# HKUST-Aerial-Robotics/MIND

Measured on AMD Instinct MI355X. Metric: sim steps/sec (whole node) + scenario-tree nodes expanded/sec, AV2 demo scenes, higher is better.
Workload: dtype f32-class (bf16 hi+mid+lo split operands = 24 significand bits, six products, fp32 accumulate) pair kernel + ActorNet, f32 elsewhere in the predictor, f64 iLQR

## Files before the change

include/mind_hip.h:

```cpp
#ifndef MIND_HIP_H
#define MIND_HIP_H

#include <stddef.h>
#include <stdint.h>

#ifdef __cplusplus
extern "C" {
#endif

#define MIND_OK 0
#define MIND_EINVAL (-1)
#define MIND_ENOMEM (-2)
#define MIND_EHIP (-3)
#define MIND_ESTATE (-4)
#define MIND_ENOTFOUND (-5)

typedef struct mind_ctx mind_ctx;

int mind_ctx_create(int device, void *stream, mind_ctx **out);
int mind_ctx_destroy(mind_ctx *ctx);
const char *mind_last_error_string(mind_ctx *ctx);
int mind_ctx_synchronize(mind_ctx *ctx);

typedef struct {
// ... 84 lines not shown
int mind_debug_aime_book(int pred_len, int max_depth, int max_rounds, int n_agents, int world, int rank, int force, int n_rounds, const int *dec_len,
                         const float *dec, int n_tokens, int bytes_per_pair, int plan_chunk_mb, int per_scene, long long *out, int cap, char *msg,
                         int msg_cap);

int mind_debug_wait_word(const unsigned *word, unsigned want, double timeout_s, double (*clock)(void *user), void *user, int spins_per_look);

int mind_debug_actor_lw_plan(int n_actors, int np, int chunk, long long *out_launches, int cap, long long *out_info);

int mind_debug_token_lw_plan(int n_tokens, int mode, int chunk, long long *out_launches, int cap, long long *out_info);

int mind_debug_pack_conv_frag(const float *w, int co, int ci, int ksz, uint32_t *out, size_t cap);

int mind_debug_pack(const char *what, const float *w, int a, int b, int c, float *out, size_t cap);
int mind_debug_weight_image(const mind_tensor_desc *tensors, int n_tensors, float *blob, size_t blob_cap, char *names, size_t names_cap,
                            long long *entries, int entries_cap, long long *out_info, char *msg, int msg_cap);
int mind_debug_weight_bind(const mind_tensor_desc *tensors, int n_tensors, const char *drop, char *msg, int msg_cap);

int mind_debug_trig(mind_ctx *ctx, const double *x, int n, double *out);

int mind_debug_dec_scene(mind_ctx *ctx, const float *rows, int n_scenes, int form, float *Cout, float *cls, int reps, float *ms);

int mind_debug_set_layers(mind_ctx *ctx, int n);
int64_t mind_debug_read(mind_ctx *ctx, const char *name, float *host, int64_t max_floats);

typedef struct {
  int n_nodes;
  const int32_t *parent;
  const float *prob;
  int n_agents;
  const float *agent_mean;
  const float *agent_cov;
  const double *field;
  const double *node_w;
} mind_cost_tree;

typedef struct {
  double dt, wheelbase;
  double w_des_state[6];
  double w_state_con[6];
  double state_lower[6], state_upper[6];
  double w_ctrl[2];
  double w_tgt, w_ego, w_ego_cov_offset, w_exo, w_exo_cov_offset, w_exo_cost_offset;
  double grid_res; int grid_w, grid_h;
  int max_iter;
} mind_ilqr_cfg;

// ... 362 lines not shown
```

mind_amd/_lib.py:

```python
import ctypes as C
import os

_HERE = os.path.dirname(os.path.abspath(__file__))
LIB_PATH = os.environ.get("MIND_HIP_LIB", os.path.join(_HERE, "libmind_hip.so"))

WAIT_CLOCK = C.CFUNCTYPE(C.c_double, C.c_void_p)
MIND_OK = 0
MIND_EINVAL, MIND_ENOMEM, MIND_EHIP, MIND_ESTATE, MIND_ENOTFOUND = -1, -2, -3, -4, -5


class TensorDesc(C.Structure):
    _fields_ = [("name", C.c_char_p), ("data", C.POINTER(C.c_float)), ("numel", C.c_int64)]


class SceneBatch(C.Structure):
    _fields_ = [("n_scenes", C.c_int), ("actor_off", C.POINTER(C.c_int32)), ("lane_off", C.POINTER(C.c_int32)),
                ("actors", C.c_void_p), ("lanes", C.c_void_p), ("lane_feat", C.c_void_p),
                ("actor_ctrs", C.c_void_p), ("actor_vecs", C.c_void_p), ("lane_ctrs", C.c_void_p),
                ("lane_vecs", C.c_void_p), ("rpe", C.POINTER(C.c_void_p)), ("tgt_nodes", C.c_void_p),
                ("tgt_rpe", C.c_void_p)]


class PredOut(C.Structure):
    _fields_ = [("cls", C.c_void_p), ("reg", C.c_void_p), ("vel", C.c_void_p), ("lane_feat", C.c_void_p),
# ... 177 lines not shown
                ("n_agents", C.c_int), ("n_trees", C.c_int), ("best", C.c_int), ("n_expanded", C.c_int), ("n_rounds", C.c_int), ("n_traj_nodes", C.c_int),
                ("costs", C.POINTER(C.c_double)), ("aime_s", C.c_double), ("ilqr_s", C.c_double), ("total_s", C.c_double),
                ("tot", LoopTotals)]


PLANNER_EGO_KEY = -(1 << 63)


class PlannerDesc(C.Structure):
    _fields_ = [("time_ahead", C.c_double), ("min_vel", C.c_float), ("dist_thres", C.c_float), ("max_depth", C.c_int), ("max_rounds", C.c_int),
                ("pred_len", C.c_int), ("prob_floor", C.c_float), ("cfg_warm", C.c_void_p), ("cfg_full", C.c_void_p), ("speculative", C.c_int),
                ("ego_type_slot", C.c_int)]


class PlannerOut(C.Structure):
    _fields_ = [("n_plans", C.c_longlong),
                ("n_agents", C.c_int), ("n_trees", C.c_int), ("best", C.c_int), ("n_expanded", C.c_int), ("n_rounds", C.c_int), ("n_traj_nodes", C.c_int),
                ("costs", C.POINTER(C.c_double)), ("ctrl", C.c_double * 2), ("aime_s", C.c_double), ("ilqr_s", C.c_double), ("total_s", C.c_double),
                ("tot", LoopTotals)]


EXPORTS = ["mind_ctx_create", "mind_ctx_destroy", "mind_last_error_string", "mind_ctx_synchronize",
           "mind_weights_load", "mind_predict_batch", "mind_last_fusion_stats", "mind_last_actor_stats", "mind_debug_actor_lw_plan", "mind_last_token_stats", "mind_last_token_stage_ms", "mind_debug_token_lw_plan", "mind_set_profiling", "mind_debug_launch_times", "mind_debug_launch_clock",
           "mind_ilqr_solve_trees", "mind_ilqr_contingency", "mind_ilqr_solve_fields", "mind_cost_eval", "mind_ilqr_score_trees", "mind_ilqr_gains", "mind_ilqr_policy_rollouts", "mind_lane_dist_field", "mind_aime_world", "mind_aime_rebase", "mind_debug_aime_decide", "mind_debug_set_layers",
           "mind_debug_read", "mind_set_pair_precision", "mind_get_pair_precision", "mind_debug_pack_bfrag", "mind_debug_pack_conv_frag", "mind_debug_pack", "mind_debug_weight_image", "mind_debug_weight_bind", "mind_debug_pair_schedule", "mind_debug_predict_choice", "mind_debug_ilqr_plan", "mind_debug_aime_book", "mind_set_tuning", "mind_get_tuning", "mind_debug_tuning", "mind_debug_live_handles", "mind_last_ilqr_stats", "mind_aime_plan", "mind_last_ilqr_profile", "mind_eval_traj_trees", "mind_last_ilqr_trace", "mind_ilqr_contingency_begin", "mind_ilqr_finish", "mind_fill_tracks", "mind_ilqr_contingency_begin_plan", "mind_debug_trig", "mind_aime_plan_begin", "mind_aime_plan_poll", "mind_aime_plan_finish", "mind_ctx_busy", "mind_ilqr_finish_plan", "mind_debug_dec_scene",
           "mind_set_exchange", "mind_last_exchange_stats", "mind_debug_wait_word",
           "mind_predict_batch_aux", "mind_set_decoder_basis", "mind_get_decoder_basis", "mind_curve_eval", "mind_debug_curve_basis",
           "mind_audit_plan", "mind_audit_episode", "mind_debug_box_clearance",
           "mind_forecast_score", "mind_debug_forecast_score",
           "mind_audit_road_plan", "mind_audit_road_episode", "mind_debug_road_margin",
           "mind_audit_ttc", "mind_debug_box_ttc",
           "mind_loop_create", "mind_loop_destroy", "mind_loop_reset", "mind_loop_advance", "mind_loop_state", "mind_loop_last_plan", "mind_loop_export",
           "mind_planner_create", "mind_planner_destroy", "mind_planner_reset", "mind_planner_observe", "mind_planner_set_lanes", "mind_planner_set_target_lane",
           "mind_planner_set_solve_lane", "mind_planner_set_eval_lane", "mind_planner_plan", "mind_planner_last_plan", "mind_planner_export"]

EXCHANGE_FN = C.CFUNCTYPE(C.c_int, C.c_void_p, C.c_int, C.c_void_p, C.c_void_p, C.c_int64)
XCHG_ALLGATHER, XCHG_ALLREDUCE, XCHG_ALLTOALLV = 0, 1, 2

_lib = None


def load():
    global _lib
    if _lib is not None:
        return _lib
    if not os.path.exists(LIB_PATH):
        raise ImportError(f"{LIB_PATH} is missing: the HIP extension must be built (hipcc --offload-arch=gfx950); "
# ... 71 lines not shown
    lib.mind_debug_live_handles.argtypes = []
    lib.mind_last_ilqr_stats.argtypes = [C.c_void_p, C.POINTER(C.c_float), C.POINTER(C.c_int), C.POINTER(C.c_int)]
    lib.mind_last_ilqr_profile.argtypes = [C.c_void_p, C.POINTER(C.c_double)]
    lib.mind_last_ilqr_trace.argtypes = [C.c_void_p, C.c_int, C.c_int, C.POINTER(C.c_double), C.c_int, C.POINTER(C.c_int)]
    lib.mind_eval_traj_trees.argtypes = [C.POINTER(C.c_double), C.POINTER(C.c_double), C.POINTER(C.c_int32), C.c_int, C.c_void_p, C.c_int, C.c_int,
                                         C.c_double, C.POINTER(C.c_double)]
    lib.mind_get_pair_precision.argtypes = [C.c_void_p]
    lib.mind_debug_pack_bfrag.argtypes = [C.POINTER(C.c_float), C.c_int, C.POINTER(C.c_uint32)]
    lib.mind_debug_pair_schedule.argtypes = [C.POINTER(C.c_int), C.POINTER(C.c_int), C.c_int, C.c_int, C.c_int, C.POINTER(C.c_int), C.c_int, C.POINTER(C.c_int)]
    lib.mind_debug_predict_choice.argtypes = [C.POINTER(C.c_char_p), C.POINTER(C.c_int), C.c_int, C.c_int, C.c_int, C.c_int, C.POINTER(C.c_int), C.POINTER(C.c_int),
                                              C.c_int, C.POINTER(C.c_longlong), C.c_int]
    lib.mind_debug_ilqr_plan.argtypes = [C.POINTER(C.c_char_p), C.POINTER(C.c_int), C.c_int, C.c_int, C.c_int, C.c_int, C.POINTER(C.c_int), C.POINTER(C.c_int32),
                                         C.POINTER(C.c_longlong), C.c_int, C.POINTER(C.c_int)]
    lib.mind_debug_wait_word.argtypes = [C.POINTER(C.c_uint), C.c_uint, C.c_double, WAIT_CLOCK, C.c_void_p, C.c_int]
    lib.mind_debug_aime_book.argtypes = [C.c_int] * 8 + [C.POINTER(C.c_int), C.POINTER(C.c_float)] + [C.c_int] * 4 + [C.POINTER(C.c_longlong), C.c_int, C.c_char_p, C.c_int]
    lib.mind_debug_trig.argtypes = [C.c_void_p, C.POINTER(C.c_double), C.c_int, C.POINTER(C.c_double)]
    lib.mind_debug_pack_conv_frag.argtypes = [C.POINTER(C.c_float), C.c_int, C.c_int, C.c_int, C.POINTER(C.c_uint32), C.c_size_t]
    lib.mind_debug_pack.argtypes = [C.c_char_p, C.POINTER(C.c_float), C.c_int, C.c_int, C.c_int, C.POINTER(C.c_float), C.c_size_t]
    lib.mind_debug_weight_image.argtypes = [C.POINTER(TensorDesc), C.c_int, C.POINTER(C.c_float), C.c_size_t, C.c_char_p, C.c_size_t,
                                            C.POINTER(C.c_longlong), C.c_int, C.POINTER(C.c_longlong), C.c_char_p, C.c_int]
    lib.mind_debug_weight_bind.argtypes = [C.POINTER(TensorDesc), C.c_int, C.c_char_p, C.c_char_p, C.c_int]
    lib.mind_debug_dec_scene.argtypes = [C.c_void_p, C.POINTER(C.c_float), C.c_int, C.c_int, C.POINTER(C.c_float), C.POINTER(C.c_float), C.c_int, C.POINTER(C.c_float)]
    lib.mind_debug_set_layers.argtypes = [C.c_void_p, C.c_int]
    lib.mind_debug_read.argtypes = [C.c_void_p, C.c_char_p, C.POINTER(C.c_float), C.c_int64]
    lib.mind_set_exchange.argtypes = [C.c_void_p, C.c_int, C.c_int, EXCHANGE_FN, C.c_void_p, C.c_int]
    lib.mind_last_exchange_stats.argtypes = [C.c_void_p, C.POINTER(C.c_longlong), C.POINTER(C.c_longlong)]
    lib.mind_loop_create.argtypes = [C.c_void_p, C.POINTER(LoopDesc), C.POINTER(C.c_void_p)]
    lib.mind_loop_destroy.argtypes = [C.c_void_p]
    lib.mind_loop_reset.argtypes = [C.c_void_p]
    lib.mind_loop_advance.argtypes = [C.c_void_p, C.c_int, C.c_double, C.c_longlong, C.POINTER(LoopOut)]
    lib.mind_loop_state.argtypes = [C.c_void_p, C.POINTER(LoopOut)]
    lib.mind_loop_last_plan.argtypes = [C.c_void_p, C.POINTER(AimePlanOut)] + [C.POINTER(C.c_void_p)] * 6 + [C.c_void_p]
    lib.mind_loop_export.argtypes = [C.c_void_p, C.c_int, C.POINTER(C.c_int), C.c_void_p, C.c_void_p, C.c_void_p]
    lib.mind_planner_create.argtypes = [C.c_void_p, C.POINTER(PlannerDesc), C.POINTER(C.c_void_p)]
    lib.mind_planner_destroy.argtypes = [C.c_void_p]
    lib.mind_planner_reset.argtypes = [C.c_void_p]
    lib.mind_planner_observe.argtypes = [C.c_void_p, C.c_int, C.c_void_p, C.c_int, C.c_void_p, C.c_void_p, C.c_void_p]
    lib.mind_planner_set_lanes.argtypes = [C.c_void_p, C.c_int, C.c_void_p, C.c_void_p]
    lib.mind_planner_set_target_lane.argtypes = [C.c_void_p, C.c_int, C.c_void_p, C.c_void_p]
    lib.mind_planner_set_solve_lane.argtypes = [C.c_void_p, C.c_int, C.c_void_p, C.c_double]
    lib.mind_planner_set_eval_lane.argtypes = [C.c_void_p, C.c_int, C.c_void_p, C.c_int]
    lib.mind_planner_plan.argtypes = [C.c_void_p, C.c_void_p, C.c_void_p, C.POINTER(PlannerOut)]
    lib.mind_planner_last_plan.argtypes = [C.c_void_p, C.POINTER(AimePlanOut)] + [C.POINTER(C.c_void_p)] * 6 + [C.c_void_p]
    lib.mind_planner_export.argtypes = [C.c_void_p, C.c_int, C.POINTER(C.c_int), C.c_void_p, C.c_void_p, C.c_void_p]
    lib.mind_audit_plan.argtypes = [C.c_void_p, C.POINTER(AuditBox), C.c_double, C.POINTER(CostTree), C.c_int, C.c_int, C.POINTER(C.c_double),
                                    C.POINTER(AuditPlanOut)]
# ... 28 lines not shown
                      "xcd_lanes5", "dec_actor", "dec_np", "fp32_dec", "split_dec", "want_mw", "mw_blocks", "cls_on_side", "tgt_wait_first",
                      "dec_head_ra", "dec_chain_g")
PAIR_PREC = ("f32", "bf16x3", "bf16", "bf16x6")


def predict_choice(knobs, prec, scenes, n_cu=256, have_side=True):
    lib = load()
    names = (C.c_char_p * max(1, len(knobs)))(*[k.encode() for k in knobs])
    vals = (C.c_int * max(1, len(knobs)))(*[int(v) for v in knobs.values()])
    sa = (C.c_int * len(scenes))(*[a for a, _ in scenes])
    sl = (C.c_int * len(scenes))(*[l for _, l in scenes])
    cap = 32 + 6 * len(scenes)
    out = (C.c_longlong * cap)()
    n = lib.mind_debug_predict_choice(names, vals, len(knobs), PAIR_PREC.index(prec) if isinstance(prec, str) else prec, n_cu, int(have_side),
                                      sa, sl, len(scenes), out, cap)
    if n == MIND_EINVAL:
        return None
    assert 0 < n <= cap and out[0] == 32 and n == 32 + 6 * out[1], n
    d = dict(zip(PRED_CHOICE_FIELDS, out[:32]))
    d["runs"] = [tuple(out[32 + 6 * i:38 + 6 * i]) for i in range(out[1])]
    return d


def dec_scene(lib, ctx, rows, form, reps=1, timed=False):
    import numpy as np
    rows = np.ascontiguousarray(rows, np.float32)
    B = rows.shape[0]
    assert rows.shape == (B, 128)
    fp = C.POINTER(C.c_float)
    cout, cls, ms = np.empty((B, 6, 128), np.float32), np.empty((B, 6), np.float32), np.zeros(reps, np.float32)
    check(lib, ctx, lib.mind_debug_dec_scene(ctx, rows.ctypes.data_as(fp), B, int(form), cout.ctypes.data_as(fp), cls.ctypes.data_as(fp), reps,
                                             ms.ctypes.data_as(fp) if timed else None), "mind_debug_dec_scene")
    return (cout, cls, ms) if timed else (cout, cls)


def knobs():
    lib = load()
    name, env, val = C.c_char_p(), C.c_char_p(), C.c_int()
    rows = []
    while not rows or len(rows) < n:
        n = lib.mind_debug_tuning(len(rows), None, None, 0, C.byref(name), C.byref(env), C.byref(val))
        assert n > 0, n
        rows.append((name.value.decode(), env.value.decode() if env.value else None, val.value))
    return rows


# ... 279 lines not shown
```

mind_amd/csrc/fusion_kernels.hip:

```cpp
#include <hip/hip_runtime.h>
#include <stdint.h>

#include "pair_common.h"

#define D_ 128
#define LDS_WAE 0
#define LDS_WAP 16384
#define LDS_STAGE 32768
#define LDS_PTAB (LDS_STAGE + PAIR_WAVES * STAGE_FLOATS)
#define LDS_SVEC (LDS_PTAB + PAIR_WAVES * 128)
#define LDS_VT (LDS_SVEC + PAIR_WAVES * 136)
#define LDS_RT (LDS_VT + VT_SIZE)
#define LDS_TOTAL (LDS_RT + 1024)

#define LDS_FENCE() asm volatile("s_waitcnt lgkmcnt(0)" ::: "memory")

__device__ __forceinline__ void gemm128(frag8 &acc, const float *wa, const frag8 &bsrc, int lane) {
  int lo = lane * 4;
  OPAQUE(lo);
  const float *wl = wa + lo;
  f32x4 c0 = *(const f32x4 *)(wl + (0 * 8 + 0) * 256);
  f32x4 c1 = *(const f32x4 *)(wl + (1 * 8 + 0) * 256);
#pragma unroll
  for (int st = 0; st < 32; ++st) {
// ... 626 lines not shown
  TT(7);
#ifdef MIND_TOKEN_TRACE
  if (blockIdx.x == 0 && tid == 0)
    printf("[k_token mode %d ntok %d] cycles: load %lld cw %lld combine %lld Wv %lld Wo+LN2 %lld FFN+LN3 %lld S,T,q %lld QK %lld\n", mode, n_tok,
           tt_[0], tt_[1], tt_[2], tt_[3], tt_[4], tt_[5], tt_[6], tt_[7]);
#endif
}

template <int TPW>
__global__ __launch_bounds__(TT_THREADS) __attribute__((amdgpu_waves_per_eu(4, 4))) void k_token(const TokMeta *__restrict__ meta, int n_tok, int mode,
                                                      const float *__restrict__ actor_feat,
                                                      const float *__restrict__ lane_feat, float *__restrict__ x,
                                                      const float *__restrict__ part, float *__restrict__ ST,
                                                      float *__restrict__ QK, TokWeights W) {
  k_token_body<TPW, false>(meta, n_tok, mode, actor_feat, lane_feat, x, part, ST, QK, W);
}
__global__ __launch_bounds__(TT_THREADS) __attribute__((amdgpu_waves_per_eu(2, 2))) void k_token_m(const TokMeta *__restrict__ meta, int n_tok, int mode,
                                                      const float *__restrict__ actor_feat,
                                                      const float *__restrict__ lane_feat, float *__restrict__ x,
                                                      const float *__restrict__ part, float *__restrict__ ST,
                                                      float *__restrict__ QK, TokWeights W) {
  k_token_body<TOK_TPW_SMALL, true>(meta, n_tok, mode, actor_feat, lane_feat, x, part, ST, QK, W);
}
```

mind_amd/csrc/mind_hip.hip:

```cpp
#include <hip/hip_runtime.h>

#include <cmath>
#include <cstdarg>
#include <cstdio>
#include <cstdlib>
#include <algorithm>
#include <cstring>
#include <map>
#include <memory>
#include <string>
#include <thread>
#include <atomic>
#include <functional>
#include <vector>

#include "../../include/mind_hip.h"
#include "encdec_kernels.hip"
#include "fusion_kernels.hip"
#include "pair_bf16_kernels.hip"
#include "pair_tile_kernels.hip"
#include "pair_tile6_kernels.hip"
#include "token_mfma_kernels.hip"
#include "actor_mfma_kernels.hip"
#include "actor_lw_kernels.hip"
// ... 149 lines not shown
  Event ev_rows;
  std::vector<const double *> il_trace_dev;
  std::vector<int> il_trace_its;
  int il_trace_cap = 0, il_trace_phases = 0;
  double il_prof[9] = {0, 0, 0, 0, 0, 0, 0, 0, 0};
  long long n_ilqr_fallbacks = 0;
  int n_pair_launch = 0;
  float pair_ms = 0.f;
  double pairs_done = 0.0;
  std::vector<Event> ev;
  bool ev_defer = false;
  std::vector<Event> ev_pool;
  size_t ev_pool_used = 0;
  std::vector<size_t> ev_pending;
  int wall_khz = 0;
  LcRing lc;
  DevBuf lc_dev;
  Pinned lc_host;
  double lc_carry_ms[LC_KINDS] = {0, 0, 0};
  int lc_carry_n[LC_KINDS] = {0, 0, 0};
  std::vector<float> lc_last[LC_KINDS], ev_last[LC_KINDS];
  int n_cu = 256;
  int debug_layers = 6;
  int last_ntok = 0;
  size_t il_dbg[6] = {0, 0, 0, 0, 0, 0};
  long long last_edge_pairs = 0;
  int last_slots = 0, last_A = 0, last_B = 0;
};

static int fail(mind_ctx *c, int code, const char *fmt, ...) {
  char buf[512];
  va_list ap;
  va_start(ap, fmt);
  vsnprintf(buf, sizeof(buf), fmt, ap);
  va_end(ap);
  if (c) c->err = buf;
  return code;
}

#define HIPCHK(c, call)                                                                        \
  do {                                                                                         \
    hipError_t e_ = (call);                                                                    \
    if (e_ != hipSuccess)                                                                      \
      return fail(c, MIND_EHIP, "%s failed: %s (%s:%d)", #call, hipGetErrorString(e_), __FILE__, __LINE__); \
  } while (0)

// ... 977 lines not shown
```

mind_amd/csrc/pred_choice.h:

```cpp
#pragma once
#include <vector>

#include "tuning.h"
#include "dec_chain.h"

static inline int pred_mfma_parts(const PredTuning &t, int pair_prec) {
  return (pair_prec == 3 || (pair_prec == 1 && t.actor_np == 6)) ? 6 : (pair_prec == 1 ? 3 : 1);
}

static inline bool pred_edge_tiled(const PredTuning &t, int pair_prec) { return pair_prec == 3 || (pair_prec != 0 && t.pair_tile); }

static inline int pred_edge_pair_bytes(const PredTuning &t, int pair_prec) { return pred_edge_tiled(t, pair_prec) && pair_prec == 2 ? 256 : 512; }

enum PredActorForm { PRED_ACTOR_VALU = 0, PRED_ACTOR_F32 = 1, PRED_ACTOR_MFMA = 2, PRED_ACTOR_LW = 3 };
enum PredPairFamily { PRED_PAIR_F32 = 0, PRED_PAIR_BF = 1, PRED_PAIR_T = 2, PRED_PAIR_T6 = 3 };
enum PredDecActor { PRED_DEC_ONE = 0, PRED_DEC_SPLIT = 1, PRED_DEC_MFMA = 2 };

struct PredTokRun {
  int t0, n, kind;
  bool layerwise;
  bool small, merged;
};

struct PredChoice {
  int np = 1;
  int actor_form = PRED_ACTOR_VALU, actor_arg = 0, actor_grid = 0, actor_chunk = 0, actor_chunks = 1, actor_launches = 1;
  int qsplit = 0, qk_stride = 1024;
  bool tiled = false, edge_bf16 = false;
  std::vector<PredTokRun> tok_runs;
  int tok_chunk = 0;
  bool tok_lw = false;
  int last_tok_chunks = 0;
  int pair_family = PRED_PAIR_F32, pair_np = 0;
  bool l5_jobs5 = false;
  int xcd_lanes = 1, xcd_lanes5 = 1;
  int dec_actor = PRED_DEC_ONE;
  int dec_head_ra = RA;
  bool fp32_dec = true, split_dec = false, want_mw = false, cls_side = false;
  int mw_blocks = 0;
  int dec_chain_g = 0;
  bool tgt_wait_first = false;
};

static PredChoice pred_choose(const PredTuning &t, int pair_prec, int n_cu, bool have_side, int n_scenes, const int *scene_actors, const int *scene_lanes) {
  PredChoice ch;
  int A = 0;
  for (int b = 0; b < n_scenes; ++b) A += scene_actors[b];
  ch.np = pred_mfma_parts(t, pair_prec);

  ch.actor_grid = A;
  if (t.actor_f32 && A >= (pair_prec == 0 ? t.actor_f32_pair_min : t.actor_f32_min)) {
    ch.actor_form = PRED_ACTOR_F32; ch.actor_arg = 2; ch.actor_grid = (A + 1) / 2;
  } else if (pair_prec == 0 && t.actor_f32 && t.enc_mfma) {
    ch.actor_form = PRED_ACTOR_F32; ch.actor_arg = 1;
  } else if (pair_prec == 0 || !t.enc_mfma) {
    ch.actor_form = PRED_ACTOR_VALU;
  } else if (A >= t.actor_lw_min) {
    ch.actor_form = PRED_ACTOR_LW; ch.actor_arg = ch.np;
    ch.actor_chunk = t.actor_lw_chunk > 0 ? t.actor_lw_chunk : LW_CHUNK;
    ch.actor_chunks = (A + ch.actor_chunk - 1) / ch.actor_chunk;
    ch.actor_grid = ch.actor_chunks;
    ch.actor_launches = ch.actor_chunks * (1 + 2 * LW_NSTAGE);
  } else {
    ch.actor_form = PRED_ACTOR_MFMA; ch.actor_arg = ch.np;
  }

  ch.qsplit = pair_prec == 3 ? 48 : pair_prec != 0 ? 16 : 0;
  ch.qk_stride = pair_prec == 3 ? P6_QK_STRIDE : 1024;
  ch.tiled = pred_edge_tiled(t, pair_prec);
  ch.edge_bf16 = pred_edge_pair_bytes(t, pair_prec) == 256;

  ch.tok_chunk = t.tok_lw_chunk > 0 ? t.tok_lw_chunk : TL_CHUNK;
  long long njobs = 0, njobs5 = 0;
  int t0 = 0;
  for (int b = 0; b < n_scenes; ++b) {
    const int N = scene_actors[b] + scene_lanes[b] + 1;
    const int kind = t.tok_mfma ? 1 : (pair_prec != 0 && pair_prec != 3 && t.tok_bf_min_n > 0 && N >= t.tok_bf_min_n) ? 2 : N >= t.tok_lw_min_n ? 1 : 0;
    if (!ch.tok_runs.empty() && ch.tok_runs.back().kind == kind) ch.tok_runs.back().n += N;
    else ch.tok_runs.push_back({t0, N, kind, false, false, false});
    t0 += N;
    njobs += (long long)N * pair_column_splits(N);
    njobs5 += (long long)(scene_actors[b] + 1) * pair_column_splits(N);
  }
  for (PredTokRun &r : ch.tok_runs) {
    r.layerwise = r.kind == 1 && r.n >= t.tok_lw_min;
    r.small = r.kind == 0 && r.n <= t.tok_small_max;
    r.merged = r.small && t.tok_merge;
    if (r.layerwise) {
      ch.tok_lw = true;
      ch.last_tok_chunks += (r.n + ch.tok_chunk - 1) / ch.tok_chunk;
    }
  }

  ch.pair_family = pair_prec == 0 ? PRED_PAIR_F32 : pair_prec == 3 ? PRED_PAIR_T6 : ch.tiled ? PRED_PAIR_T : PRED_PAIR_BF;
  ch.pair_np = (ch.pair_family == PRED_PAIR_T || ch.pair_family == PRED_PAIR_BF) ? (pair_prec == 1 ? 3 : 1) : 0;
  ch.l5_jobs5 = ch.tiled;
  ch.xcd_lanes = pair_xcd_lanes(t.xcd_order, n_scenes, pair_grid(njobs, n_cu));
  ch.xcd_lanes5 = pair_xcd_lanes(t.xcd_order, n_scenes, pair_grid(njobs5, n_cu));

  ch.fp32_dec = pair_prec == 0 || !t.enc_mfma || A < t.dec_mfma_min;
  ch.split_dec = ch.fp32_dec && have_side && t.dec_overlap;
  ch.dec_actor = ch.split_dec ? PRED_DEC_SPLIT : ch.fp32_dec ? PRED_DEC_ONE : PRED_DEC_MFMA;
  if (ch.split_dec) ch.dec_head_ra = t.dec_head_ra ? t.dec_head_ra : A <= n_cu ? 1 : (A + 1) / 2 <= n_cu ? 2 : RA;
  ch.mw_blocks = ((n_scenes + 7) / 8) * 8 * DEC_MW_G;
  ch.want_mw = t.dec_mw && ch.mw_blocks <= n_cu;
  ch.cls_side = ch.split_dec && t.dec_cls_side;
  ch.dec_chain_g = (t.dec_mw || t.dec_cls_side) ? 0 : dc_choose_g(n_scenes, n_cu);
  ch.tgt_wait_first = have_side && !t.tgt_side;
  return ch;
}
// ... 1 lines not shown
```

mind_amd/csrc/predict.hip:

```cpp
__global__ void k_tokpos(const TokMeta *__restrict__ meta, int n_tok, const float *__restrict__ actr,
                         const float *__restrict__ avec, const float *__restrict__ lctr,
                         const float *__restrict__ lvec, float *__restrict__ tokpos) {
  const int t = blockIdx.x * blockDim.x + threadIdx.x;
  if (t >= n_tok) return;
  const TokMeta m = meta[t];
  float4 o = make_float4(0.f, 0.f, 0.f, 0.f);
  if (m.type == 0 && actr) o = make_float4(actr[m.src * 2], actr[m.src * 2 + 1], avec[m.src * 2], avec[m.src * 2 + 1]);
  if (m.type == 1 && lctr) o = make_float4(lctr[m.src * 2], lctr[m.src * 2 + 1], lvec[m.src * 2], lvec[m.src * 2 + 1]);
  ((float4 *)tokpos)[t] = o;
}

struct PairTables {
  std::vector<TokMeta> meta;
  std::vector<PairJob> jobs, jobs5;
  std::vector<int> actor_row, actor_scene, cls_row, scene_n;
  long long edge_pairs = 0, edge_pairs_t = 0;
  int ntok = 0, slot = 0;
  double pairs_full = 0, pairs_l5 = 0;
};

static void pair_tables_build(int Bn, const int *scene_actors, const int *scene_lanes, bool xcd_order, int n_cu, PairTables &T) {
  int A = 0;
  for (int b = 0; b < Bn; ++b) A += scene_actors[b];
  T.actor_row.assign(A, 0); T.actor_scene.assign(A, 0); T.cls_row.assign(Bn, 0); T.scene_n.assign(Bn, 0);
// ... 78 lines not shown
                                         const int *scene_actors, const int *scene_lanes, int n_scenes, long long *out, int cap) {
  if (n_knobs < 0 || (n_knobs > 0 && (!knob_names || !knob_values)) || pair_prec < 0 || pair_prec > 3 || n_cu <= 0 || !scene_actors || !scene_lanes ||
      n_scenes <= 0 || cap < 0 || (cap > 0 && !out))
    return MIND_EINVAL;
  PredTuning t;
  const TnRefs own{&t, nullptr, nullptr};
  for (int k = 0; k < n_knobs; ++k)
    if (!knob_names[k] || !tn_set(own, knob_names[k], knob_values[k])) return MIND_EINVAL;
  for (int b = 0; b < n_scenes; ++b)
    if (scene_actors[b] <= 0 || scene_lanes[b] < 0) return MIND_EINVAL;
  const PredChoice ch = pred_choose(t, pair_prec, n_cu, have_side != 0, n_scenes, scene_actors, scene_lanes);
  const bool mfma_dec = ch.dec_actor == PRED_DEC_MFMA;
  const long long head[PRED_CHOICE_HEADER] = {
      PRED_CHOICE_HEADER, (long long)ch.tok_runs.size(), ch.np, ch.actor_form, ch.actor_arg, ch.actor_grid, ch.actor_chunk, ch.actor_chunks,
      ch.actor_launches, ch.qsplit, ch.qk_stride, ch.tiled, ch.edge_bf16, pred_edge_pair_bytes(t, pair_prec), ch.tok_chunk, ch.tok_lw,
      ch.last_tok_chunks, ch.pair_family, ch.pair_np, ch.l5_jobs5, ch.xcd_lanes, ch.xcd_lanes5, ch.dec_actor, mfma_dec ? ch.np : 0,
      ch.fp32_dec, ch.split_dec, ch.want_mw, ch.mw_blocks, ch.cls_side && !ch.want_mw, ch.tgt_wait_first, ch.split_dec ? ch.dec_head_ra : 0, ch.dec_chain_g};
  std::vector<long long> rec(head, head + PRED_CHOICE_HEADER);
  for (const PredTokRun &r : ch.tok_runs) rec.insert(rec.end(), {r.t0, r.n, r.kind, r.layerwise, r.small, r.merged});
  for (size_t i = 0; i < rec.size() && (int)i < cap; ++i) out[i] = rec[i];
  return (int)rec.size();
}

static bool lc_on(const mind_ctx *c) { return c->profiling && c->ct.prof_clock != 0 && c->wall_khz > 0; }
static bool lc_events(const mind_ctx *c) { return c->profiling && !(c->ct.prof_clock == 1 && c->wall_khz > 0); }

static void lc_account(mind_ctx *c, const LcRecord &r, double (&ms)[LC_KINDS], int (&n)[LC_KINDS]) {
  const double t = lc_ticks_ms(lc_reduce(c->lc_host.as<LcSlot>() + c->lc.slot_of(r.block), r.grid), c->wall_khz);
  ms[r.kind] += t; n[r.kind] += 1;
  c->lc_last[r.kind].push_back((float)t);
}

static int lc_flush(mind_ctx *c, bool keep) {
  const int n = (int)c->lc.pending.size();
  if (n > 0) {
    HIPCHK(c, hipStreamSynchronize(c->stream));
    if (c->pl_copy) HIPCHK(c, hipStreamSynchronize(c->pl_copy));
    int first[2], count[2];
    const int runs = c->lc.pending_runs(0, n, first, count);
    for (int k = 0; k < runs; ++k) {
      const size_t o = c->lc.slot_of(first[k]), b = (size_t)count[k] * c->lc.block_slots * sizeof(LcSlot);
      HIPCHK(c, hipMemcpy(c->lc_host.as<LcSlot>() + o, (const LcSlot *)c->lc_dev.p + o, b, hipMemcpyDeviceToHost));
    }
    if (keep)
      for (const LcRecord &r : c->lc.pending) lc_account(c, r, c->lc_carry_ms, c->lc_carry_n);
    c->lc.drained(n);
// ... 258 lines not shown

static int pred_token_step(PredCall &p, int mode, int Lw) {
  mind_ctx *c = p.c;
  hipStream_t st = p.st;
  const size_t qk_stride = p.ch.qk_stride, tokm_lds = mind_token_mfma_lds_bytes();
  const float *actor_feat = (const float *)c->actor_feat.p, *lane_feat = p.lane_feat;
  float *part = (float *)c->part.p;
  HIPCHK(c, pred_tok_mark(p, -1));
  for (const PredTokRun &r : p.ch.tok_runs) {
    const TokMeta *m_ = (const TokMeta *)p.ts->meta.p + r.t0;
    float *x_ = p.x() + (size_t)r.t0 * 128, *ST_ = (float *)c->ST.p + (size_t)r.t0 * 256, *QK_ = (float *)c->QK.p + (size_t)r.t0 * qk_stride;
    if (r.layerwise) {
      tl_build_plan(r.n, mode, p.ch.tok_chunk, c->n_cu, c->tok_lw_plan);
      for (const TlLaunch &L : c->tok_lw_plan) {
        if (tl_launch(L, st, mode, m_, actor_feat, lane_feat, x_, part, ST_, QK_, qk_stride, c->W.tok[Lw], c->W.tokM[Lw], (float *)c->tok_lw_arena.p, p.ch.tok_chunk))
          return fail(c, MIND_ESTATE, "layer-wise token stage: a stage has no kernel");
        HIPCHK(c, pred_tok_mark(p, L.stage));
      }
      c->last_tok_launches += (int)c->tok_lw_plan.size();
      continue;
    }
    c->last_tok_launches++;
    if (r.kind == 0) {
      const int tpw = r.small ? TOK_TPW_SMALL : TOK_TPW_BIG;
      hipLaunchKernelGGL(r.small ? (r.merged ? k_token_m : k_token<TOK_TPW_SMALL>) : k_token<TOK_TPW_BIG>, dim3((r.n + tpw - 1) / tpw), dim3(TT_THREADS), 0,
                         st, m_, r.n, mode, actor_feat, lane_feat, x_, part, ST_, QK_, c->W.tok[Lw]);
    } else if (r.kind == 1) {
      hipLaunchKernelGGL(k_token_mfma<0>, dim3((r.n + TM_TOK - 1) / TM_TOK), dim3(TM_THREADS), tokm_lds, st, m_, r.n, mode, actor_feat, lane_feat, x_,
                         part, ST_, QK_, c->W.tok[Lw], c->W.tokM[Lw]);
    } else {
      hipLaunchKernelGGL(k_token_mfma<1>, dim3((r.n + TM_TOK - 1) / TM_TOK), dim3(TM_THREADS), tokm_lds, st, m_, r.n, mode, actor_feat, lane_feat, x_,
                         part, ST_, QK_, c->W.tok[Lw], c->W.tokB[Lw]);
    }
    HIPCHK(c, pred_tok_mark(p, TL_NSTAGE));
  }
  return MIND_OK;
}

static int pred_pair_layer(PredCall &p, int L) {
  mind_ctx *c = p.c;
  const PredChoice &ch = p.ch;
  const TableSet *ts = p.ts;
  const bool last = L == 5, own5 = last && ch.l5_jobs5;
  const int um = L < 4 ? 0 : (L == 4 ? 1 : 2);
  const PairJob *jl = (const PairJob *)(own5 ? ts->jobs5.p : ts->jobs.p);
  const int nj = own5 ? ts->njobs5 : ts->njobs;
  const dim3 grid(pair_grid(nj, c->n_cu)), block(PAIR_THREADS);
  float *edge = (float *)c->edge.p, *ST = (float *)c->ST.p, *QK = (float *)c->QK.p, *part = (float *)c->part.p, *tokpos = (float *)c->tokpos.p;
  const size_t ldsb = mind_pair_bf_lds_bytes();
// ... 199 lines not shown
    }
  }
  return MIND_OK;
}

extern "C" int mind_predict_batch_aux(mind_ctx *c, const mind_scene_batch *in, mind_pred_out *out, const mind_pred_aux *aux) {
  if (!c || !in || !out) return MIND_EINVAL;
  if (!c->have_weights) return fail(c, MIND_ESTATE, "weights not loaded");
  const int Bn = in->n_scenes;
  if (Bn <= 0 || !in->actor_off || !in->lane_off || !in->actors || !in->tgt_nodes || !in->tgt_rpe || !out->cls ||
      !out->reg || !out->vel)
    return fail(c, MIND_EINVAL, "null input/output pointer");
  if (!in->lanes && !in->lane_feat) return fail(c, MIND_EINVAL, "need lanes or lane_feat");
  if (!in->rpe && !(in->actor_ctrs && in->actor_vecs && in->lane_ctrs && in->lane_vecs))
    return fail(c, MIND_EINVAL, "need rpe or ctrs/vecs");
  HIPCHK(c, hipSetDevice(c->device));
  const int A = in->actor_off[Bn], Ltot = in->lane_off[Bn];
  if (A <= 0 || Ltot < 0) return fail(c, MIND_EINVAL, "empty batch");
  std::vector<int> sa(Bn), sl(Bn);
  for (int b = 0; b < Bn; ++b) {
    sa[b] = in->actor_off[b + 1] - in->actor_off[b]; sl[b] = in->lane_off[b + 1] - in->lane_off[b];
    if (sa[b] <= 0 || sl[b] < 0) return fail(c, MIND_EINVAL, "scene %d has %d agents, %d lanes", b, sa[b], sl[b]);
  }
  const PredChoice ch = pred_choose(c->pt, c->pair_prec, c->n_cu, c->side.p != nullptr, Bn, sa.data(), sl.data());
  PredCall p{c, in, out, aux, ch, Bn, A, Ltot, c->stream, c->side ? c->side.p : c->stream};
  int rc;
  if ((rc = pred_tables(p, sa.data(), sl.data()))) return rc;
  if ((rc = pred_workspaces(p))) return rc;
  if ((rc = pred_encoders(p))) return rc;
  if ((rc = pred_fusion(p))) return rc;
  if ((rc = pred_decoder(p))) return rc;
  return pred_finish(p);
}

extern "C" int mind_predict_batch(mind_ctx *c, const mind_scene_batch *in, mind_pred_out *out) { return mind_predict_batch_aux(c, in, out, nullptr); }
```

Baseline: 1931.

## Add mode-specialized small token kernels with two-token workgroups for merged runs

Adds k_token_s, a token-layer kernel templated on tokens per workgroup (2 or 4) and on the stage mask (init/epilogue/projection). Each instantiation compiles only the stages its mode needs, and weight loads are interleaved with compute to hide latency. For merged small runs, a rule picks two tokens per workgroup when that still fits within one workgroup per CU, spreading work across more CUs; otherwise it uses four. The change adds more kernel variants and LDS usage, and modes without a specialization return an error.

```diff
diff --git a/include/mind_hip.h b/include/mind_hip.h
--- a/include/mind_hip.h
+++ b/include/mind_hip.h
@@ -130,6 +130,8 @@
 
 int mind_debug_set_layers(mind_ctx *ctx, int n);
 int64_t mind_debug_read(mind_ctx *ctx, const char *name, float *host, int64_t max_floats);
+
+int mind_debug_token_form(mind_ctx *ctx, int form, int n_tok, int n_cu);
 
 typedef struct {
   int n_nodes;
diff --git a/mind_amd/_lib.py b/mind_amd/_lib.py
--- a/mind_amd/_lib.py
+++ b/mind_amd/_lib.py
@@ -223,7 +223,7 @@
 
 EXPORTS = ["mind_ctx_create", "mind_ctx_destroy", "mind_last_error_string", "mind_ctx_synchronize",
            "mind_weights_load", "mind_predict_batch", "mind_last_fusion_stats", "mind_last_actor_stats", "mind_debug_actor_lw_plan", "mind_last_token_stats", "mind_last_token_stage_ms", "mind_debug_token_lw_plan", "mind_set_profiling", "mind_debug_launch_times", "mind_debug_launch_clock",
-           "mind_ilqr_solve_trees", "mind_ilqr_contingency", "mind_ilqr_solve_fields", "mind_cost_eval", "mind_ilqr_score_trees", "mind_ilqr_gains", "mind_ilqr_policy_rollouts", "mind_lane_dist_field", "mind_aime_world", "mind_aime_rebase", "mind_debug_aime_decide", "mind_debug_set_layers",
+           "mind_ilqr_solve_trees", "mind_ilqr_contingency", "mind_ilqr_solve_fields", "mind_cost_eval", "mind_ilqr_score_trees", "mind_ilqr_gains", "mind_ilqr_policy_rollouts", "mind_lane_dist_field", "mind_aime_world", "mind_aime_rebase", "mind_debug_aime_decide", "mind_debug_set_layers", "mind_debug_token_form",
            "mind_debug_read", "mind_set_pair_precision", "mind_get_pair_precision", "mind_debug_pack_bfrag", "mind_debug_pack_conv_frag", "mind_debug_pack", "mind_debug_weight_image", "mind_debug_weight_bind", "mind_debug_pair_schedule", "mind_debug_predict_choice", "mind_debug_ilqr_plan", "mind_debug_aime_book", "mind_set_tuning", "mind_get_tuning", "mind_debug_tuning", "mind_debug_live_handles", "mind_last_ilqr_stats", "mind_aime_plan", "mind_last_ilqr_profile", "mind_eval_traj_trees", "mind_last_ilqr_trace", "mind_ilqr_contingency_begin", "mind_ilqr_finish", "mind_fill_tracks", "mind_ilqr_contingency_begin_plan", "mind_debug_trig", "mind_aime_plan_begin", "mind_aime_plan_poll", "mind_aime_plan_finish", "mind_ctx_busy", "mind_ilqr_finish_plan", "mind_debug_dec_scene",
            "mind_set_exchange", "mind_last_exchange_stats", "mind_debug_wait_word",
            "mind_predict_batch_aux", "mind_set_decoder_basis", "mind_get_decoder_basis", "mind_curve_eval", "mind_debug_curve_basis",
@@ -341,6 +341,7 @@
     lib.mind_debug_weight_bind.argtypes = [C.POINTER(TensorDesc), C.c_int, C.c_char_p, C.c_char_p, C.c_int]
     lib.mind_debug_dec_scene.argtypes = [C.c_void_p, C.POINTER(C.c_float), C.c_int, C.c_int, C.POINTER(C.c_float), C.POINTER(C.c_float), C.c_int, C.POINTER(C.c_float)]
     lib.mind_debug_set_layers.argtypes = [C.c_void_p, C.c_int]
+    lib.mind_debug_token_form.argtypes = [C.c_void_p, C.c_int, C.c_int, C.c_int]
     lib.mind_debug_read.argtypes = [C.c_void_p, C.c_char_p, C.POINTER(C.c_float), C.c_int64]
     lib.mind_set_exchange.argtypes = [C.c_void_p, C.c_int, C.c_int, EXCHANGE_FN, C.c_void_p, C.c_int]
     lib.mind_last_exchange_stats.argtypes = [C.c_void_p, C.POINTER(C.c_longlong), C.POINTER(C.c_longlong)]
@@ -415,6 +416,14 @@
     return d
 
 
+TOKEN_FORMS = ("rule", "k_token_m", "k_token_s<4>", "k_token_s<2>")
+
+
+def token_form(form, n_tok=0, n_cu=256, ctx=None):
+    n = load().mind_debug_token_form(ctx, int(form), int(n_tok), int(n_cu))
+    return None if n == MIND_EINVAL else n
+
+
 def dec_scene(lib, ctx, rows, form, reps=1, timed=False):
     import numpy as np
     rows = np.ascontiguousarray(rows, np.float32)
diff --git a/mind_amd/csrc/fusion_kernels.hip b/mind_amd/csrc/fusion_kernels.hip
--- a/mind_amd/csrc/fusion_kernels.hip
+++ b/mind_amd/csrc/fusion_kernels.hip
@@ -672,3 +672,303 @@
                                                       float *__restrict__ QK, TokWeights W) {
   k_token_body<TOK_TPW_SMALL, true>(meta, n_tok, mode, actor_feat, lane_feat, x, part, ST, QK, W);
 }
+
+template <int TP, int N>
+__device__ __forceinline__ void ksum_s(const float (&acc)[N][TP], const float (&bias)[N], float *rk, int kg, int col, int ta, float (&r)[N]) {
+  constexpr int ST = TKG * TP * 128;
+  __syncthreads();
+#pragma unroll
+  for (int n = 0; n < N; ++n)
+#pragma unroll
+    for (int t = 0; t < TP; ++t) rk[n * ST + (kg * TP + t) * 128 + col] = acc[n][t];
+  __syncthreads();
+#pragma unroll
+  for (int n = 0; n < N; ++n) {
+    const float *q = rk + n * ST;
+    r[n] = ((q[(0 * TP + ta) * 128 + col] + q[(1 * TP + ta) * 128 + col]) + (q[(2 * TP + ta) * 128 + col] + q[(3 * TP + ta) * 128 + col])) + bias[n];
+  }
+}
+
+template <int TPW, int SM>
+__device__ __forceinline__ void k_token_small_body(const TokMeta *__restrict__ meta, int n_tok, int mode, const float *__restrict__ actor_feat,
+                                                   const float *__restrict__ lane_feat, float *__restrict__ x, const float *__restrict__ part,
+                                                   float *__restrict__ ST, float *__restrict__ QK, const TokWeights &W) {
+  static_assert(TPW == 2 || TPW == 4, "two or four tokens per workgroup");
+  constexpr bool INIT = (SM & 1) != 0, EPI = (SM & 2) != 0, PRO = (SM & 4) != 0;
+  __shared__ __attribute__((aligned(16))) float xs[TPW][132];
+  __shared__ __attribute__((aligned(16))) float tmp[TPW][260];
+  __shared__ __attribute__((aligned(16))) float mb[TPW][8][132];
+  __shared__ float rk[3 * TKG * TPW * 128];
+  __shared__ float rd[TKG * 2 * 2];
+  __shared__ float cw[TPW][8][8];
+  const int tid = threadIdx.x, kg = tid >> 7, col = tid & 127;
+  const int tok0 = blockIdx.x * TPW;
+  const int nt = min(TPW, n_tok - tok0);
+  const int ta = TPW == 4 ? kg : (kg & 1);
+  const bool own = kg < TPW, va = own && ta < nt;
+  constexpr bool DEEP = TPW == 2;
+  constexpr int NH = TPW == 4 ? 8 : 4;
+  const int h0 = TPW == 4 ? 0 : (kg >> 1) * 4;
+  const int ct = tid >> 3, chd = tid & 7;
+  const bool cwt = tid < TPW * 8;
+#ifdef MIND_TOKEN_TRACE
+  long long tt_[10] = {0, 0, 0, 0, 0, 0, 0, 0, 0, 0}, tq_ = clock64();
+#endif
+
+  int tya = 2, srca = 0, nsa = 0, slota = 0, nsc = 0, slotc = 0;
+  if (ta < nt) {
+    const TokMeta m = meta[tok0 + ta];
+    tya = m.type; srca = m.src; slota = m.slot0;
+    nsa = ((mode & 8) && !(m.flags & 1)) ? 0 : min(m.nsplit, 8);
+  }
+  if (cwt && ct < nt) {
+    const TokMeta m = meta[tok0 + ct];
+    slotc = m.slot0;
+    nsc = ((mode & 8) && !(m.flags & 1)) ? 0 : min(m.nsplit, 8);
+  }
+  float xv = 0.f;
+  if (!INIT && va) xv = x[(size_t)(tok0 + ta) * 128 + col];
+  float wpa[32], wpl[32], wv[32], wo[32], w1a[32], w1b[32], w2[64], ws[32], wt[32], wq[32], wk[2][16];
+  float b_pa = 0.f, b_pl = 0.f, b_v = 0.f, b_o = 0.f, g_2 = 0.f, be_2 = 0.f, b_1a = 0.f, b_1b = 0.f, b_2 = 0.f, g_3 = 0.f, be_3 = 0.f, b_m = 0.f, b_q = 0.f;
+  float ga = 0.f, gl = 0.f, ba = 0.f, bl = 0.f;
+  if constexpr (INIT) {
+    mv_load<128>(wpa, W.WpaT, 128, col, kg);
+    mv_load<128>(wpl, W.WplT, 128, col, kg);
+    b_pa = W.bpa[col]; b_pl = W.bpl[col];
+    ga = W.gpa[col]; gl = W.gpl[col]; ba = W.bepa[col]; bl = W.bepl[col];
+  }
+  if constexpr (EPI) {
+    mv_load<128>(wv, W.WvT, 128, col, kg);
+    b_v = W.bv[col];
+  }
+#define TOK_S_LOAD_STQ()                                  \
+  do {                                                    \
+    mv_load<128>(ws, W.WsT, 128, col, kg);                \
+    mv_load<128>(wt, W.WtT, 128, col, kg);                \
+    mv_load<128>(wq, W.WqT, 128, col, kg);                \
+    b_m = W.bm[col]; b_q = W.bq[col];                     \
+  } while (0)
+  if constexpr (PRO && !EPI && DEEP) TOK_S_LOAD_STQ();
+
+  float pm[8], pl[8], pv[8][NH];
+  if constexpr (EPI) {
+    if (cwt) {
+#pragma unroll
+      for (int s = 0; s < 8; ++s) {
+        pm[s] = 0.f; pl[s] = 0.f;
+        if (s < nsc) {
+          const float *ps = part + (size_t)(slotc + s) * PART_STRIDE;
+          pm[s] = ps[chd]; pl[s] = ps[8 + chd];
+        }
+      }
+    }
+#pragma unroll
+    for (int s = 0; s < 8; ++s) {
+#pragma unroll
+      for (int h = 0; h < NH; ++h) pv[s][h] = 0.f;
+      if (s < nsa) {
+        const float *ps = part + (size_t)(slota + s) * PART_STRIDE + 16 + col;
+#pragma unroll
+        for (int h = 0; h < NH; ++h) pv[s][h] = ps[(h0 + h) * 128];
+      }
+    }
+  }
+
+  if constexpr (INIT) {
+    float fa = 0.f;
+    if (ta < nt) {
+      if (tya == 0) fa = actor_feat[(size_t)srca * 128 + col];
+      else if (tya == 1) fa = lane_feat[(size_t)srca * 128 + col];
+    }
+    if (own) tmp[ta][col] = fa;
+    __syncthreads();
+    float ac2[2][TPW], r[2];
+    mv_fma<128, TPW>(ac2[0], wpa, &tmp[0][0], 260, kg);
+    mv_fma<128, TPW>(ac2[1], wpl, &tmp[0][0], 260, kg);
+    if constexpr (PRO && !EPI && !DEEP) TOK_S_LOAD_STQ();
+    const float bs[2] = {b_pa, b_pl};
+    ksum_s<TPW, 2>(ac2, bs, rk, kg, col, ta, r);
+    float p0 = tya == 0 ? r[0] : r[1];
+    {
+      float s0 = p0, s1 = 0.f;
+      gsum2(s0, s1, rd, kg, tid);
+      const float d0 = p0 - s0 * (1.0f / 128.0f);
+      s0 = d0 * d0; s1 = 0.f;
+      gsum2(s0, s1, rd, kg, tid);
+      p0 = fmaxf(d0 * (1.0f / sqrtf(s0 * (1.0f / 128.0f) + 1e-5f)) * (tya == 0 ? ga : gl) + (tya == 0 ? ba : bl), 0.f);
+      if (tya == 2) p0 = 0.f;
+    }
+    if (own) xs[ta][col] = p0;
+    __syncthreads();
+  } else {
+    if (own) xs[ta][col] = xv;
+    __syncthreads();
+  }
+  TT(0);
+  if constexpr (EPI) {
+    if (cwt) {
+      float wgt[8];
+      float M = -INFINITY;
+#pragma unroll
+      for (int s = 0; s < 8; ++s)
+        if (s < nsc) M = fmaxf(M, pm[s]);
+      float L = 0.f;
+#pragma unroll
+      for (int s = 0; s < 8; ++s) {
+        wgt[s] = 0.f;
+        if (s < nsc) {
+          const float e = expf(pm[s] - M);
+          wgt[s] = e;
+          L += e * pl[s];
+        }
+      }
+      const float inv = 1.0f / L;
+#pragma unroll
+      for (int s = 0; s < 8; ++s)
+        if (s < nsc) wgt[s] *= inv;
+#pragma unroll
+      for (int s = 0; s < 8; ++s) cw[ct][chd][s] = wgt[s];
+    }
+#define TOK_S_LOAD_WO() do { mv_load<128>(wo, W.WoT, 128, col, kg); b_o = W.bo[col]; g_2 = W.g2[col]; be_2 = W.b2[col]; } while (0)
+#define TOK_S_LOAD_W1() do { mv_load<128>(w1a, W.W1T, 256, col, kg); mv_load<128>(w1b, W.W1T, 256, 128 + col, kg); b_1a = W.b1[col]; b_1b = W.b1[128 + col]; } while (0)
+#define TOK_S_LOAD_W2() do { mv_load<256>(w2, W.W2T, 128, col, kg); b_2 = W.bb2[col]; g_3 = W.g3[col]; be_3 = W.b3[col]; } while (0)
+    if constexpr (DEEP) TOK_S_LOAD_WO();
+    __syncthreads();
+    TT(1);
+    {
+      float v[NH];
+#pragma unroll
+      for (int h = 0; h < NH; ++h) v[h] = 0.f;
+#pragma unroll
+      for (int s = 0; s < 8; ++s)
+        if (s < nsa) {
+#pragma unroll
+          for (int h = 0; h < NH; ++h) v[h] = fmaf(cw[ta][h0 + h][s], pv[s][h], v[h]);
+        }
+#pragma unroll
+      for (int h = 0; h < NH; ++h) mb[ta][h0 + h][col] = v[h];
+    }
+    if constexpr (DEEP) TOK_S_LOAD_W1(); else TOK_S_LOAD_WO();
+    __syncthreads();
+    TT(2);
+    {
+      float acc[1][TPW], r[1];
+      mv_fma<128, TPW>(acc[0], wv, &mb[0][col >> 4][0], 8 * 132, kg);
+      if constexpr (DEEP) TOK_S_LOAD_W2(); else TOK_S_LOAD_W1();
+      const float bs[1] = {b_v};
+      ksum_s<TPW, 1>(acc, bs, rk, kg, col, ta, r);
+      if (own) tmp[ta][col] = r[0];
+      __syncthreads();
+    }
+    TT(3);
+    {
+      float acc[1][TPW], r[1];
+      mv_fma<128, TPW>(acc[0], wo, &tmp[0][0], 260, kg);
+      const float bs[1] = {b_o};
+      ksum_s<TPW, 1>(acc, bs, rk, kg, col, ta, r);
+      float p0 = r[0] + xs[ta][col], p1 = 0.f;
+      ln2tok(p0, p1, g_2, be_2, rd, kg, tid);
+      __syncthreads();
+      if (own) xs[ta][col] = p0;
+      __syncthreads();
+    }
+    TT(4);
+    {
+      float ac2[2][TPW], r[2];
+      mv_fma<128, TPW>(ac2[0], w1a, &xs[0][0], 132, kg);
+      mv_fma<128, TPW>(ac2[1], w1b, &xs[0][0], 132, kg);
+      if constexpr (PRO && DEEP) TOK_S_LOAD_STQ();
+      if constexpr (!DEEP) TOK_S_LOAD_W2();
+      const float bs[2] = {b_1a, b_1b};
+      ksum_s<TPW, 2>(ac2, bs, rk, kg, col, ta, r);
+      if (own) { tmp[ta][col] = fmaxf(r[0], 0.f); tmp[ta][128 + col] = fmaxf(r[1], 0.f); }
+      __syncthreads();
+      float acc[1][TPW], q[1];
+      mv_fma<256, TPW>(acc[0], w2, &tmp[0][0], 260, kg);
+      if constexpr (PRO && !DEEP) TOK_S_LOAD_STQ();
+      const float b2s[1] = {b_2};
+      ksum_s<TPW, 1>(acc, b2s, rk, kg, col, ta, q);
+      float p0 = q[0] + xs[ta][col], p1 = 0.f;
+      ln2tok(p0, p1, g_3, be_3, rd, kg, tid);
+      __syncthreads();
+      if (own) xs[ta][col] = p0;
+      __syncthreads();
+    }
+  }
+  TT(5);
+  if (va) x[(size_t)(tok0 + ta) * 128 + col] = xs[ta][col];
+
+  if constexpr (PRO) {
+#define TOK_S_LOAD_WK()                                                                                 \
+  _Pragma("unroll") for (int hh = 0; hh < 2; ++hh)                                                      \
+    _Pragma("unroll") for (int d = 0; d < 16; ++d) wk[hh][d] = W.Wk[(size_t)((2 * kg + hh) * 16 + d) * 128 + col]
+    if constexpr (DEEP) { TOK_S_LOAD_WK(); }
+    {
+      float ac3[3][TPW], q[3];
+      mv_fma<128, TPW>(ac3[0], ws, &xs[0][0], 132, kg);
+      mv_fma<128, TPW>(ac3[1], wt, &xs[0][0], 132, kg);
+      mv_fma<128, TPW>(ac3[2], wq, &xs[0][0], 132, kg);
+      if constexpr (!DEEP) { TOK_S_LOAD_WK(); }
+      const float bs[3] = {0.f, b_m, b_q};
+      ksum_s<TPW, 3>(ac3, bs, rk, kg, col, ta, q);
+      if (va) { ST[(size_t)(tok0 + ta) * 256 + col] = q[0]; ST[(size_t)(tok0 + ta) * 256 + 128 + col] = q[1]; }
+      if (own) tmp[ta][col] = q[2];
+    }
+    __syncthreads();
+    TT(6);
+#pragma unroll
+    for (int hh = 0; hh < 2; ++hh) {
+      const int hd = 2 * kg + hh;
+      float acc[TPW];
+#pragma unroll
+      for (int t = 0; t < TPW; ++t) acc[t] = 0.f;
+#pragma unroll
+      for (int d = 0; d < 16; d += 4)
+#pragma unroll
+        for (int t = 0; t < TPW; ++t) {
+          const float4 xq = *reinterpret_cast<const float4 *>(&tmp[t][hd * 16 + d]);
+          acc[t] = fmaf(wk[hh][d], xq.x, acc[t]);
+          acc[t] = fmaf(wk[hh][d + 1], xq.y, acc[t]);
+          acc[t] = fmaf(wk[hh][d + 2], xq.z, acc[t]);
+          acc[t] = fmaf(wk[hh][d + 3], xq.w, acc[t]);
+        }
+      if (mode & 16) {
+        const int g = col >> 5, qq = (col >> 2) & 3, i = 4 * ((col >> 4) & 1) + (col & 3);
+        const int idx = ((g * 32) + hd * 4 + qq) * 8 + i;
+        const size_t qks = (mode & 32) ? 1536 : 1024;
+        for (int t = 0; t < nt; ++t) {
+          const float v = acc[t] * 0.25f;
+          const u32 h = pk_bf16(v, v) & 0xffffu;
+          const float r1 = v - bf_lo_f32(h);
+          const u32 l = pk_bf16(r1, 0.f) & 0xffffu;
+          unsigned short *qs = reinterpret_cast<unsigned short *>(QK + (size_t)(tok0 + t) * qks);
+          qs[idx] = (unsigned short)h;
+          qs[1024 + idx] = (unsigned short)l;
+          if (mode & 32) qs[2048 + idx] = (unsigned short)(pk_bf16(r1 - bf_lo_f32(l), 0.f) & 0xffffu);
+        }
+      } else {
+        for (int t = 0; t < nt; ++t) QK[(size_t)(tok0 + t) * 1024 + hd * 128 + col] = acc[t] * 0.25f;
+      }
+    }
+  }
+  TT(7);
+#undef TOK_S_LOAD_STQ
+#undef TOK_S_LOAD_WK
+#undef TOK_S_LOAD_WO
+#undef TOK_S_LOAD_W1
+#undef TOK_S_LOAD_W2
+#ifdef MIND_TOKEN_TRACE
+  if (blockIdx.x == 0 && tid == 0)
+    printf("[k_token_s<%d> mode %d ntok %d] cycles: load %lld cw %lld combine %lld Wv %lld Wo+LN2 %lld FFN+LN3 %lld S,T,q %lld QK %lld\n", TPW, mode, n_tok,
+           tt_[0], tt_[1], tt_[2], tt_[3], tt_[4], tt_[5], tt_[6], tt_[7]);
+#endif
+}
+
+template <int TPW, int SM>
+__global__ __launch_bounds__(TT_THREADS) __attribute__((amdgpu_waves_per_eu(2, 2))) void k_token_s(const TokMeta *__restrict__ meta, int n_tok, int mode,
+                                                      const float *__restrict__ actor_feat,
+                                                      const float *__restrict__ lane_feat, float *__restrict__ x,
+                                                      const float *__restrict__ part, float *__restrict__ ST,
+                                                      float *__restrict__ QK, TokWeights W) {
+  k_token_small_body<TPW, SM>(meta, n_tok, mode, actor_feat, lane_feat, x, part, ST, QK, W);
+}
diff --git a/mind_amd/csrc/mind_hip.hip b/mind_amd/csrc/mind_hip.hip
--- a/mind_amd/csrc/mind_hip.hip
+++ b/mind_amd/csrc/mind_hip.hip
@@ -195,6 +195,7 @@
   std::vector<float> lc_last[LC_KINDS], ev_last[LC_KINDS];
   int n_cu = 256;
   int debug_layers = 6;
+  int debug_tok_form = 0;
   int last_ntok = 0;
   size_t il_dbg[6] = {0, 0, 0, 0, 0, 0};
   long long last_edge_pairs = 0;
diff --git a/mind_amd/csrc/pred_choice.h b/mind_amd/csrc/pred_choice.h
--- a/mind_amd/csrc/pred_choice.h
+++ b/mind_amd/csrc/pred_choice.h
@@ -20,7 +20,15 @@
   int t0, n, kind;
   bool layerwise;
   bool small, merged;
+  int form;
 };
+
+enum PredTokForm { PRED_TOK_RULE = 0, PRED_TOK_M = 1, PRED_TOK_S4 = 2, PRED_TOK_S2 = 3 };
+
+static inline int pred_tok_form(int forced, int n_tok, int n_cu) {
+  if (forced == PRED_TOK_M || forced == PRED_TOK_S4 || forced == PRED_TOK_S2) return forced;
+  return (n_tok + 1) / 2 <= n_cu ? PRED_TOK_S2 : PRED_TOK_S4;
+}
 
 struct PredChoice {
   int np = 1;
@@ -42,7 +50,8 @@
   bool tgt_wait_first = false;
 };
 
-static PredChoice pred_choose(const PredTuning &t, int pair_prec, int n_cu, bool have_side, int n_scenes, const int *scene_actors, const int *scene_lanes) {
+static PredChoice pred_choose(const PredTuning &t, int pair_prec, int n_cu, bool have_side, int n_scenes, const int *scene_actors, const int *scene_lanes,
+                              int tok_form = PRED_TOK_RULE) {
   PredChoice ch;
   int A = 0;
   for (int b = 0; b < n_scenes; ++b) A += scene_actors[b];
@@ -77,7 +86,7 @@
     const int N = scene_actors[b] + scene_lanes[b] + 1;
     const int kind = t.tok_mfma ? 1 : (pair_prec != 0 && pair_prec != 3 && t.tok_bf_min_n > 0 && N >= t.tok_bf_min_n) ? 2 : N >= t.tok_lw_min_n ? 1 : 0;
     if (!ch.tok_runs.empty() && ch.tok_runs.back().kind == kind) ch.tok_runs.back().n += N;
-    else ch.tok_runs.push_back({t0, N, kind, false, false, false});
+    else ch.tok_runs.push_back({t0, N, kind, false, false, false, 0});
     t0 += N;
     njobs += (long long)N * pair_column_splits(N);
     njobs5 += (long long)(scene_actors[b] + 1) * pair_column_splits(N);
@@ -86,6 +95,7 @@
     r.layerwise = r.kind == 1 && r.n >= t.tok_lw_min;
     r.small = r.kind == 0 && r.n <= t.tok_small_max;
     r.merged = r.small && t.tok_merge;
+    r.form = r.merged ? pred_tok_form(tok_form, r.n, n_cu) : 0;
     if (r.layerwise) {
       ch.tok_lw = true;
       ch.last_tok_chunks += (r.n + ch.tok_chunk - 1) / ch.tok_chunk;
diff --git a/mind_amd/csrc/predict.hip b/mind_amd/csrc/predict.hip
--- a/mind_amd/csrc/predict.hip
+++ b/mind_amd/csrc/predict.hip
@@ -124,6 +124,15 @@
   return (int)rec.size();
 }
 
+extern "C" int mind_debug_token_form(mind_ctx *c, int form, int n_tok, int n_cu) {
+  if (form < PRED_TOK_RULE || form > PRED_TOK_S2 || n_tok < 0 || (n_tok > 0 && n_cu <= 0)) return MIND_EINVAL;
+  if (c) c->debug_tok_form = form;
+  if (n_tok == 0) return form;
+  const int one = 1, lanes = n_tok - 2;
+  const PredChoice ch = pred_choose(PredTuning(), 3, n_cu, true, 1, &one, &lanes, form);
+  return ch.tok_runs[0].form;
+}
+
 static bool lc_on(const mind_ctx *c) { return c->profiling && c->ct.prof_clock != 0 && c->wall_khz > 0; }
 static bool lc_events(const mind_ctx *c) { return c->profiling && !(c->ct.prof_clock == 1 && c->wall_khz > 0); }
 
@@ -428,9 +437,18 @@
     }
     c->last_tok_launches++;
     if (r.kind == 0) {
-      const int tpw = r.small ? TOK_TPW_SMALL : TOK_TPW_BIG;
-      hipLaunchKernelGGL(r.small ? (r.merged ? k_token_m : k_token<TOK_TPW_SMALL>) : k_token<TOK_TPW_BIG>, dim3((r.n + tpw - 1) / tpw), dim3(TT_THREADS), 0,
-                         st, m_, r.n, mode, actor_feat, lane_feat, x_, part, ST_, QK_, c->W.tok[Lw]);
+      const int tpw = r.form == PRED_TOK_S2 ? 2 : r.small ? TOK_TPW_SMALL : TOK_TPW_BIG;
+      auto *kern = r.small ? (r.merged ? k_token_m : k_token<TOK_TPW_SMALL>) : k_token<TOK_TPW_BIG>;
+      if (r.form == PRED_TOK_S2 || r.form == PRED_TOK_S4) {
+        const bool two = r.form == PRED_TOK_S2;
+        switch (mode & 7) {
+          case 5: kern = two ? k_token_s<2, 5> : k_token_s<TOK_TPW_SMALL, 5>; break;
+          case 6: kern = two ? k_token_s<2, 6> : k_token_s<TOK_TPW_SMALL, 6>; break;
+          case 2: kern = two ? k_token_s<2, 2> : k_token_s<TOK_TPW_SMALL, 2>; break;
+          default: return fail(c, MIND_ESTATE, "token step: mode %d has no small-launch kernel", mode);
+        }
+      }
+      hipLaunchKernelGGL(kern, dim3((r.n + tpw - 1) / tpw), dim3(TT_THREADS), 0, st, m_, r.n, mode, actor_feat, lane_feat, x_, part, ST_, QK_, c->W.tok[Lw]);
     } else if (r.kind == 1) {
       hipLaunchKernelGGL(k_token_mfma<0>, dim3((r.n + TM_TOK - 1) / TM_TOK), dim3(TM_THREADS), tokm_lds, st, m_, r.n, mode, actor_feat, lane_feat, x_,
                          part, ST_, QK_, c->W.tok[Lw], c->W.tokM[Lw]);
@@ -676,7 +694,7 @@
     sa[b] = in->actor_off[b + 1] - in->actor_off[b]; sl[b] = in->lane_off[b + 1] - in->lane_off[b];
     if (sa[b] <= 0 || sl[b] < 0) return fail(c, MIND_EINVAL, "scene %d has %d agents, %d lanes", b, sa[b], sl[b]);
   }
-  const PredChoice ch = pred_choose(c->pt, c->pair_prec, c->n_cu, c->side.p != nullptr, Bn, sa.data(), sl.data());
+  const PredChoice ch = pred_choose(c->pt, c->pair_prec, c->n_cu, c->side.p != nullptr, Bn, sa.data(), sl.data(), c->debug_tok_form);
   PredCall p{c, in, out, aux, ch, Bn, A, Ltot, c->stream, c->side ? c->side.p : c->stream};
   int rc;
   if ((rc = pred_tables(p, sa.data(), sl.data()))) return rc;
```

Result: faster. 1978, median of 6 (+2.5%).
